# vressegu/sdeflow-light

Hardware: AMD Instinct MI355X
Metric: score-matching train steps/sec (+ reverse-SDE sample steps/sec) (higher is better)
Workload: dtype f32

## Files before the change

sdeflow_light_amd/csrc/attention_train_kernels.hip:

```cpp
#include "attention_common.h"

template <int CT, int QT, int KB, int NW = 4, bool MH = false>
__global__ void __launch_bounds__(64 * NW) k_attn_dual_fwd(const float* __restrict__ qkv, float* __restrict__ att,
                                                        float* __restrict__ lse, float* __restrict__ rbar, int T, int nqb,
                                                        int64_t Bp, float scale, int nh) {
  constexpr int C = 16 * CT, KP = C + 4, KT = KB / 16, NT = 64 * NW;
  constexpr int NV = (KB * C / 4) / NT;
  static_assert(NV >= 1 && (KB * C / 4) % NT == 0, "key block does not divide over the workgroup's threads");
  extern __shared__ __attribute__((aligned(16))) float atd_lds[];
  float* Ks = atd_lds;
  float* Kd = Ks + KB * KP;
  float* Vs = Kd + KB * KP;
  float* Vd = Vs + KB * KP;
  const int tid = threadIdx.x, w = tid >> 6, lane = tid & 63, il = lane & 15, q = lane >> 4;
  const int64_t NP = MH ? Bp * nh : Bp;
  int pr, qb;
  {
    const int full = (int)(NP / 8) * 8 * nqb, b = blockIdx.x;
    if (b < full) { const int loc = b >> 3; pr = (loc / nqb) * 8 + (b & 7); qb = loc % nqb; }
    else { const int r = b - full; pr = (int)(NP / 8) * 8 + r / nqb; qb = r % nqb; }
  }
  const AttnHead H = attn_head<MH, C>(pr, nh);
  const int LD = H.LD, LA = H.LA, smp = H.smp;
  const float* bp = qkv + (size_t)smp * T * LD + H.qcol;
  const float* bt = bp + (size_t)Bp * T * LD;
  const int q0 = (qb * NW + w) * 16 * QT;

  f32x4 qf[QT][CT], qd[QT][CT], o[QT][CT], od[QT][CT];
  float m[QT], l[QT], rr[QT];
#pragma unroll
  for (int qt = 0; qt < QT; ++qt) {
#pragma unroll
    for (int g = 0; g < CT; ++g) {
      const size_t off = (size_t)(q0 + 16 * qt + il) * LD + 16 * g + 4 * q;
      qf[qt][g] = *reinterpret_cast<const f32x4*>(bp + off);
      qd[qt][g] = *reinterpret_cast<const f32x4*>(bt + off);
      o[qt][g] = f32x4{0, 0, 0, 0};
      od[qt][g] = f32x4{0, 0, 0, 0};
    }
    m[qt] = -INFINITY; l[qt] = 0.f; rr[qt] = 0.f;
  }

  f32x4 pk[NV], pkd[NV], pv[NV], pvd[NV];
  auto gload = [&](int kb) __attribute__((always_inline)) {
#pragma unroll
    for (int i = 0; i < NV; ++i) {
      const int idx = tid + NT * i, key = idx / (C / 4), c4 = idx - key * (C / 4);
      const size_t off = (size_t)(kb * KB + key) * LD + 4 * c4;
      pk[i] = *reinterpret_cast<const f32x4*>(bp + off + C);
      pv[i] = *reinterpret_cast<const f32x4*>(bp + off + 2 * C);
      pkd[i] = *reinterpret_cast<const f32x4*>(bt + off + C);
      pvd[i] = *reinterpret_cast<const f32x4*>(bt + off + 2 * C);
    }
  };
  gload(0);
  const int nkb = T / KB;
  for (int kb = 0; kb < nkb; ++kb) {
    __syncthreads();
#pragma unroll
    for (int i = 0; i < NV; ++i) {
      const int idx = tid + NT * i, key = idx / (C / 4), c4 = idx - key * (C / 4);
      *reinterpret_cast<f32x4*>(Ks + key * KP + 4 * c4) = pk[i];
      *reinterpret_cast<f32x4*>(Kd + key * KP + 4 * c4) = pkd[i];
      *reinterpret_cast<f32x4*>(Vs + key * KP + 4 * c4) = pv[i];
      *reinterpret_cast<f32x4*>(Vd + key * KP + 4 * c4) = pvd[i];
    }
    __syncthreads();
    if (kb + 1 < nkb) gload(kb + 1);

    f32x4 s[QT][KT], sd[QT][KT];
#pragma unroll
    for (int kt = 0; kt < KT; ++kt) {
#pragma unroll
      for (int qt = 0; qt < QT; ++qt) { s[qt][kt] = f32x4{0, 0, 0, 0}; sd[qt][kt] = f32x4{0, 0, 0, 0}; }
#pragma unroll
      for (int g = 0; g < CT; ++g) {
        const f32x4 a = *reinterpret_cast<const f32x4*>(Ks + (16 * kt + il) * KP + 16 * g + 4 * q);
        const f32x4 ad = *reinterpret_cast<const f32x4*>(Kd + (16 * kt + il) * KP + 16 * g + 4 * q);
#pragma unroll
        for (int r = 0; r < 4; ++r)
#pragma unroll
          for (int qt = 0; qt < QT; ++qt) {
            s[qt][kt] = mfma16(a[r], qf[qt][g][r], s[qt][kt]);
            sd[qt][kt] = mfma16(a[r], qd[qt][g][r], sd[qt][kt]);
            sd[qt][kt] = mfma16(ad[r], qf[qt][g][r], sd[qt][kt]);
          }
      }
    }
#pragma unroll
    for (int qt = 0; qt < QT; ++qt) {
      float mb = -INFINITY;
#pragma unroll
      for (int kt = 0; kt < KT; ++kt)
#pragma unroll
        for (int r = 0; r < 4; ++r) { s[qt][kt][r] *= scale; mb = fmaxf(mb, s[qt][kt][r]); }
      mb = fmaxf(mb, __shfl_xor(mb, 16, 64));
      mb = fmaxf(mb, __shfl_xor(mb, 32, 64));
      const float mn = fmaxf(m[qt], mb);
      const float alpha = expf(m[qt] - mn);
      m[qt] = mn;
      float ls = 0.f, lr = 0.f;
#pragma unroll
      for (int kt = 0; kt < KT; ++kt)
#pragma unroll
        for (int r = 0; r < 4; ++r) {
          const float p = expf(s[qt][kt][r] - mn);
          const float wv = p * (sd[qt][kt][r] * scale);
          s[qt][kt][r] = p; sd[qt][kt][r] = wv;
          ls += p; lr += wv;
        }
      l[qt] = l[qt] * alpha + ls;
      rr[qt] = rr[qt] * alpha + lr;
#pragma unroll
      for (int ct = 0; ct < CT; ++ct) { o[qt][ct] *= alpha; od[qt][ct] *= alpha; }
    }
#pragma unroll
    for (int kt = 0; kt < KT; ++kt)
#pragma unroll
      for (int ct = 0; ct < CT; ++ct) {
        float a[4], ad[4];
#pragma unroll
        for (int r = 0; r < 4; ++r) {
          a[r] = Vs[(16 * kt + 4 * q + r) * KP + 16 * ct + il];
          ad[r] = Vd[(16 * kt + 4 * q + r) * KP + 16 * ct + il];
        }
#pragma unroll
        for (int r = 0; r < 4; ++r)
#pragma unroll
          for (int qt = 0; qt < QT; ++qt) {
            o[qt][ct] = mfma16(a[r], s[qt][kt][r], o[qt][ct]);
            od[qt][ct] = mfma16(a[r], sd[qt][kt][r], od[qt][ct]);
            od[qt][ct] = mfma16(ad[r], s[qt][kt][r], od[qt][ct]);
          }
      }
  }
#pragma unroll
  for (int qt = 0; qt < QT; ++qt) {
    float lt = l[qt], rt = rr[qt];
    lt += __shfl_xor(lt, 16, 64); lt += __shfl_xor(lt, 32, 64);
    rt += __shfl_xor(rt, 16, 64); rt += __shfl_xor(rt, 32, 64);
    const float inv = 1.0f / lt, rb = rt * inv;
    const size_t row = (size_t)smp * T + q0 + 16 * qt + il;
    float* orow = att + row * LA + H.acol;
    float* drow = att + ((size_t)Bp * T + row) * LA + H.acol;
#pragma unroll
    for (int ct = 0; ct < CT; ++ct) {
      const f32x4 ov = o[qt][ct] * inv;
      *reinterpret_cast<f32x4*>(orow + 16 * ct + 4 * q) = ov;
      *reinterpret_cast<f32x4*>(drow + 16 * ct + 4 * q) = od[qt][ct] * inv - ov * rb;
    }
    if (q == 0) {
      const size_t sr = (size_t)pr * T + q0 + 16 * qt + il;
      lse[sr] = m[qt] + logf(lt); rbar[sr] = rb;
    }
  }
}

template <bool MH = false>
__global__ void __launch_bounds__(256) k_attn_dual_delta(const float* __restrict__ att, const float* __restrict__ datt,
                                                          const float* __restrict__ rbar, float* __restrict__ cc,
                                                          float* __restrict__ de, int64_t rows, int C, int T, int nh) {
  const int64_t row = (int64_t)blockIdx.x * 16 + (threadIdx.x >> 4);
  const int sl = threadIdx.x & 15;
  float c = 0.f, d = 0.f;
  if (row < rows) {
    const size_t off = MH ? attn_mh_row(row / T, row % T, T, C, nh) : (size_t)row * C;
    const float* o = att + off;
    const float* g = datt + off;
    const float* od = att + (size_t)rows * C + off;
    const float* gd = datt + (size_t)rows * C + off;
    for (int c4 = sl; c4 < C / 4; c4 += 16) {
      const f32x4 ov = *reinterpret_cast<const f32x4*>(o + 4 * c4), gv = *reinterpret_cast<const f32x4*>(g + 4 * c4);
      const f32x4 odv = *reinterpret_cast<const f32x4*>(od + 4 * c4), gdv = *reinterpret_cast<const f32x4*>(gd + 4 * c4);
#pragma unroll
      for (int r = 0; r < 4; ++r) { c += gdv[r] * ov[r]; d += gv[r] * ov[r] + gdv[r] * odv[r]; }
    }
  }
#pragma unroll
  for (int s = 8; s > 0; s >>= 1) { c += __shfl_xor(c, s, 16); d += __shfl_xor(d, s, 16); }
  if (row < rows && sl == 0) { cc[row] = c; de[row] = d - rbar[row] * c; }
}

template <int CT, int KG, bool ACC = false, bool MH = false>
__global__ void __launch_bounds__(128 * KG) k_attn_dual_bwd(const float* __restrict__ qkv, const float* __restrict__ datt,
                                                        const float* __restrict__ stats ,
                                                        const float* __restrict__ ccde ,
                                                        float* __restrict__ dqkv, float* __restrict__ slab, int T, int nkg,
                                                        int kseq, int ks, int64_t Bp, float scale, int nh) {
  constexpr int C = 16 * CT, KP = C + 4, KB = 16 * KG, DP = KB + 4, QB = 32, NT = 128 * KG;
  constexpr int NK = (KB * C / 4 + NT - 1) / NT;
  constexpr bool KFULL = (KB * C / 4) % NT == 0;
  constexpr int NQ = (QB * C / 4 + NT - 1) / NT;
  constexpr bool QFULL = (QB * C / 4) % NT == 0;
  static_assert(NK >= 1 && NQ >= 1 && (KFULL || NK == 1) && (QFULL || NQ == 1), "tiles do not divide over the workgroup");
  const int64_t NP = MH ? Bp * nh : Bp;
  extern __shared__ __attribute__((aligned(16))) float atb_lds[];
  float* Ks = atb_lds;
  float* Kd = Ks + KB * KP;
  float* Vs = Kd + KB * KP;
  float* Vd = Vs + KB * KP;
  float* Qs = Vd + KB * KP;
  float* Qd = Qs + QB * KP;
  float* Gs = Qd + QB * KP;
  float* Gd = Gs + QB * KP;
  float* St = Gd + QB * KP;
  float* dS0 = St + 4 * QB;
  const int tid = threadIdx.x, w = tid >> 6, lane = tid & 63, il = lane & 15, q = lane >> 4;
  const int qs = w & 1, kg = w >> 1;
  int pr, kgi;
  {
    const int full = (int)(NP / 8) * 8 * nkg, b = blockIdx.x;
    if (b < full) { const int loc = b >> 3; pr = (loc / nkg) * 8 + (b & 7); kgi = loc % nkg; }
    else { const int r = b - full; pr = (int)(NP / 8) * 8 + r / nkg; kgi = r % nkg; }
  }
  const AttnHead H = attn_head<MH, C>(pr, nh);
  const int LD = H.LD, LA = H.LA, smp = H.smp;
  const int kb = kgi * kseq + ks;
  const size_t half_qkv = (size_t)Bp * T * LD, half_att = (size_t)Bp * T * LA;
  const float* bp = qkv + (size_t)smp * T * LD + H.qcol;
  const float* gp = datt + (size_t)smp * T * LA + H.acol;
  const size_t srow0 = (size_t)pr * T;

#pragma unroll
  for (int i = 0; i < NK; ++i) {
    const int idx = tid + NT * i, key = idx / (C / 4), c4 = idx - key * (C / 4);
    if (!KFULL && idx >= KB * C / 4) break;
    const size_t off = (size_t)(kb * KB + key) * LD + 4 * c4;
    *reinterpret_cast<f32x4*>(Ks + key * KP + 4 * c4) = *reinterpret_cast<const f32x4*>(bp + off + C);
    *reinterpret_cast<f32x4*>(Vs + key * KP + 4 * c4) = *reinterpret_cast<const f32x4*>(bp + off + 2 * C);
    *reinterpret_cast<f32x4*>(Kd + key * KP + 4 * c4) = *reinterpret_cast<const f32x4*>(bp + half_qkv + off + C);
    *reinterpret_cast<f32x4*>(Vd + key * KP + 4 * c4) = *reinterpret_cast<const f32x4*>(bp + half_qkv + off + 2 * C);
  }

  f32x4 dk[CT], dkd[CT], dv[CT], dvd[CT];
#pragma unroll
  for (int ct = 0; ct < CT; ++ct) dk[ct] = dkd[ct] = dv[ct] = dvd[ct] = f32x4{0, 0, 0, 0};

  f32x4 pq[NQ], pqd[NQ], pg[NQ], pgd[NQ];
  float pst = 0.f;
  auto gload = [&](int qb) __attribute__((always_inline)) {
#pragma unroll
    for (int i = 0; i < NQ; ++i) {
      const int idx = tid + NT * i, qr = idx / (C / 4), c4 = idx - qr * (C / 4);
      if (!QFULL && idx >= QB * C / 4) break;
      const size_t row = (size_t)(qb * QB + qr);
      pq[i] = *reinterpret_cast<const f32x4*>(bp + row * LD + 4 * c4);
      pqd[i] = *reinterpret_cast<const f32x4*>(bp + half_qkv + row * LD + 4 * c4);
      pg[i] = *reinterpret_cast<const f32x4*>(gp + row * LA + 4 * c4);
      pgd[i] = *reinterpret_cast<const f32x4*>(gp + half_att + row * LA + 4 * c4);
    }
    if (tid < 4 * QB) {
      const int which = tid >> 5, qr = tid & 31;
      const size_t o = (size_t)(which & 1) * (size_t)NP * T + srow0 + (size_t)qb * QB + qr;
      pst = which < 2 ? stats[o] : ccde[o];
    }
  };
  gload(0);
  const int nqb = T / QB;
  for (int qb = 0; qb < nqb; ++qb) {
    float* dS = dS0 + (qb & 1) * (2 * QB * DP);
    float* dSd = dS + QB * DP;
#pragma unroll
    for (int i = 0; i < NQ; ++i) {
      const int idx = tid + NT * i, qr = idx / (C / 4), c4 = idx - qr * (C / 4);
      if (!QFULL && idx >= QB * C / 4) break;
      *reinterpret_cast<f32x4*>(Qs + qr * KP + 4 * c4) = pq[i];
      *reinterpret_cast<f32x4*>(Qd + qr * KP + 4 * c4) = pqd[i];
      *reinterpret_cast<f32x4*>(Gs + qr * KP + 4 * c4) = pg[i];
      *reinterpret_cast<f32x4*>(Gd + qr * KP + 4 * c4) = pgd[i];
    }
    if (tid < 4 * QB) St[tid] = pst;
    __syncthreads();
    if (qb + 1 < nqb) gload(qb + 1);

    f32x4 s = {0, 0, 0, 0}, sd = {0, 0, 0, 0}, pb = {0, 0, 0, 0}, dd = {0, 0, 0, 0};
#pragma unroll
    for (int g = 0; g < CT; ++g) {
      const int ao = (16 * qs + il) * KP + 16 * g + 4 * q, bo = (16 * kg + il) * KP + 16 * g + 4 * q;
      const f32x4 aQ = *reinterpret_cast<const f32x4*>(Qs + ao), aQd = *reinterpret_cast<const f32x4*>(Qd + ao);
      const f32x4 aG = *reinterpret_cast<const f32x4*>(Gs + ao), aGd = *reinterpret_cast<const f32x4*>(Gd + ao);
      const f32x4 bK = *reinterpret_cast<const f32x4*>(Ks + bo), bKd = *reinterpret_cast<const f32x4*>(Kd + bo);
      const f32x4 bV = *reinterpret_cast<const f32x4*>(Vs + bo), bVd = *reinterpret_cast<const f32x4*>(Vd + bo);
#pragma unroll
      for (int r = 0; r < 4; ++r) {
        s = mfma16(aQ[r], bK[r], s);
        sd = mfma16(aQd[r], bK[r], sd);
        pb = mfma16(aG[r], bV[r], pb);
        dd = mfma16(aGd[r], bV[r], dd);
        sd = mfma16(aQ[r], bKd[r], sd);
        pb = mfma16(aGd[r], bVd[r], pb);
      }
      __builtin_amdgcn_sched_barrier(0);
    }
    const f32x4 L4 = *reinterpret_cast<const f32x4*>(St + 16 * qs + 4 * q);
    const f32x4 R4 = *reinterpret_cast<const f32x4*>(St + QB + 16 * qs + 4 * q);
    const f32x4 C4 = *reinterpret_cast<const f32x4*>(St + 2 * QB + 16 * qs + 4 * q);
    const f32x4 D4 = *reinterpret_cast<const f32x4*>(St + 3 * QB + 16 * qs + 4 * q);
    f32x4 p, pd, ds, dsd;
#pragma unroll
    for (int r = 0; r < 4; ++r) {
      const float sv = s[r] * scale, sdv = sd[r] * scale;
      const float pv = expf(sv - L4[r]), e = sdv - R4[r];
      p[r] = pv;
      pd[r] = pv * e;
      dsd[r] = pv * (dd[r] - C4[r]);
      ds[r] = pv * (pb[r] + dd[r] * e - C4[r] * sdv - D4[r]);
      dS[(16 * qs + 4 * q + r) * DP + 16 * kg + il] = ds[r];
      dSd[(16 * qs + 4 * q + r) * DP + 16 * kg + il] = dsd[r];
    }
#pragma unroll
    for (int ct = 0; ct < CT; ++ct) {
      float aG[4], aGd[4], aQ[4], aQd[4];
#pragma unroll
      for (int r = 0; r < 4; ++r) {
        const int o = (16 * qs + 4 * q + r) * KP + 16 * ct + il;
        aG[r] = Gs[o]; aGd[r] = Gd[o]; aQ[r] = Qs[o]; aQd[r] = Qd[o];
      }
#pragma unroll
      for (int r = 0; r < 4; ++r) {
        dv[ct] = mfma16(aG[r], p[r], dv[ct]);
        dvd[ct] = mfma16(aGd[r], p[r], dvd[ct]);
        dk[ct] = mfma16(aQ[r], ds[r], dk[ct]);
        dkd[ct] = mfma16(aQ[r], dsd[r], dkd[ct]);
        dv[ct] = mfma16(aGd[r], pd[r], dv[ct]);
        dk[ct] = mfma16(aQd[r], dsd[r], dk[ct]);
      }
      __builtin_amdgcn_sched_barrier(0);
    }
    __syncthreads();
#pragma unroll
    for (int ct = kg; ct < CT; ct += KG) {
      const size_t row = (size_t)qb * QB + 16 * qs + il;
      float* sp = slab + (((size_t)pr * nkg + kgi) * T + row) * C + 16 * ct + 4 * q;
      float* sdp = slab + (((size_t)(NP + pr) * nkg + kgi) * T + row) * C + 16 * ct + 4 * q;
      f32x4 dq = {0, 0, 0, 0}, dqd = {0, 0, 0, 0}, pdq = {0, 0, 0, 0}, pdqd = {0, 0, 0, 0};
      if (ACC) {
        pdq = *reinterpret_cast<const f32x4*>(sp);
        pdqd = *reinterpret_cast<const f32x4*>(sdp);
      }
#pragma unroll
      for (int kt = 0; kt < KG; ++kt) {
        const f32x4 b1 = *reinterpret_cast<const f32x4*>(dS + (16 * qs + il) * DP + 16 * kt + 4 * q);
        const f32x4 b2 = *reinterpret_cast<const f32x4*>(dSd + (16 * qs + il) * DP + 16 * kt + 4 * q);
        float a1[4], a2[4];
#pragma unroll
        for (int r = 0; r < 4; ++r) {
          a1[r] = Ks[(16 * kt + 4 * q + r) * KP + 16 * ct + il];
          a2[r] = Kd[(16 * kt + 4 * q + r) * KP + 16 * ct + il];
        }
#pragma unroll
        for (int r = 0; r < 4; ++r) {
          dq = mfma16(a1[r], b1[r], dq);
          dqd = mfma16(a1[r], b2[r], dqd);
          dq = mfma16(a2[r], b2[r], dq);
        }
      }
      if (ACC) { dq += pdq; dqd += pdqd; }
      *reinterpret_cast<f32x4*>(sp) = dq;
      *reinterpret_cast<f32x4*>(sdp) = dqd;
    }
  }
  __syncthreads();
  float* scratch = atb_lds;
  if (qs == 1) {
#pragma unroll
    for (int ct = 0; ct < CT; ++ct) {
      f32x4* base = reinterpret_cast<f32x4*>(scratch) + ((size_t)kg * 4 * CT + 4 * ct) * 64 + lane;
      base[0] = dk[ct]; base[64] = dkd[ct]; base[128] = dv[ct]; base[192] = dvd[ct];
    }
  }
  __syncthreads();
  if (qs == 0) {
    const size_t row = (size_t)smp * T + kb * KB + 16 * kg + il;
    float* kp_ = dqkv + row * LD + H.qcol;
    float* kt_ = dqkv + half_qkv + row * LD + H.qcol;
#pragma unroll
    for (int ct = 0; ct < CT; ++ct) {
      const f32x4* base = reinterpret_cast<const f32x4*>(scratch) + ((size_t)kg * 4 * CT + 4 * ct) * 64 + lane;
      *reinterpret_cast<f32x4*>(kp_ + C + 16 * ct + 4 * q) = (dk[ct] + base[0]) * scale;
      *reinterpret_cast<f32x4*>(kt_ + C + 16 * ct + 4 * q) = (dkd[ct] + base[64]) * scale;
      *reinterpret_cast<f32x4*>(kp_ + 2 * C + 16 * ct + 4 * q) = dv[ct] + base[128];
      *reinterpret_cast<f32x4*>(kt_ + 2 * C + 16 * ct + 4 * q) = dvd[ct] + base[192];
    }
  }
}

template <bool MH = false>
__global__ void __launch_bounds__(256) k_attn_dq_reduce(const float* __restrict__ slab, float* __restrict__ dqkv, int64_t N,
                                                         int T, int C, int nkb, float scale, int nh) {
  const int64_t total = N * T * (C / 4);
  for (int64_t i = (int64_t)blockIdx.x * 256 + threadIdx.x; i < total; i += (int64_t)gridDim.x * 256) {
    const int c4 = (int)(i % (C / 4));
    const int64_t row = i / (C / 4);
    const int64_t n = row / T, qr = row - n * T;
    const float* p = slab + ((size_t)n * nkb * T + qr) * C + 4 * c4;
    f32x4 acc = *reinterpret_cast<const f32x4*>(p);
    for (int kb = 1; kb < nkb; ++kb) acc += *reinterpret_cast<const f32x4*>(p + (size_t)kb * T * C);
    *reinterpret_cast<f32x4*>(dqkv + (MH ? attn_mh_row(n, qr, T, 3 * C, nh) : (size_t)row * 3 * C) + 4 * c4) = acc * scale;
  }
}

template <int CT, int QT, int KB, int NW, bool MH = false>
static int launch_fwd(const float* qkv, float* att, float* stats, int64_t Bp, int T, float scale, hipStream_t st, int nh = 1) {
  constexpr int C = 16 * CT;
  constexpr size_t lds = (size_t)4 * KB * (C + 4) * sizeof(float);
  static const int once = attn_allow_lds(&k_attn_dual_fwd<CT, QT, KB, NW, MH>, lds); (void)once;
  const int nqb = T / (16 * NW * QT);
  const int64_t NP = Bp * nh;
  hipLaunchKernelGGL((k_attn_dual_fwd<CT, QT, KB, NW, MH>), dim3((unsigned)(NP * nqb)), dim3(64 * NW), lds, st, qkv, att, stats,
                     stats + NP * T, T, nqb, Bp, scale, nh);
  return msgm_check_launch();
}

static inline int attn_bwd_keys(int C) { return C == 128 ? 32 : 64; }

template <int CT, int KG, bool MH = false>
static int launch_bwd(const float* qkv, const float* att, const float* datt, const float* stats, float* dqkv, int64_t Bp, int T,
                      float scale, float* ws, hipStream_t st, int nh = 1) {
  constexpr int C = 16 * CT, KP = C + 4, KB = 16 * KG;
  constexpr size_t lds_main = ((size_t)4 * KB * KP + 4 * 32 * KP + 4 * 32 + 4 * 32 * (KB + 4)) * sizeof(float);
  constexpr size_t lds_epi = (size_t)KG * 4 * CT * 64 * 4 * sizeof(float);
  constexpr size_t lds = lds_main > lds_epi ? lds_main : lds_epi;
  static_assert(lds <= 160 * 1024, "backward tiles exceed the CU's LDS");
  static const int once = attn_allow_lds(&k_attn_dual_bwd<CT, KG, false, MH>, lds) | attn_allow_lds(&k_attn_dual_bwd<CT, KG, true, MH>, lds);
  (void)once;
  const int64_t NP = Bp * nh;
  const int64_t rows = NP * T;
  const int nkb = T / KB;
  int kseq = 1;
  for (int k = 2; k > 1; k >>= 1)
    if (nkb % k == 0 && NP * (int64_t)(nkb / k) >= 1024) { kseq = k; break; }
  const int nkg = nkb / kseq;
  float* cc = ws;
  float* de = ws + rows;
  float* slab = ws + 2 * rows;
  hipLaunchKernelGGL(k_attn_dual_delta<MH>, dim3((unsigned)((rows + 15) / 16)), dim3(256), 0, st, att, datt, stats + rows, cc, de,
                     rows, C, T, nh);
  hipLaunchKernelGGL((k_attn_dual_bwd<CT, KG, false, MH>), dim3((unsigned)(NP * nkg)), dim3(128 * KG), lds, st, qkv, datt, stats, cc, dqkv,
                     slab, T, nkg, kseq, 0, Bp, scale, nh);
  for (int ks = 1; ks < kseq; ++ks)
    hipLaunchKernelGGL((k_attn_dual_bwd<CT, KG, true, MH>), dim3((unsigned)(NP * nkg)), dim3(128 * KG), lds, st, qkv, datt, stats, cc,
                       dqkv, slab, T, nkg, kseq, ks, Bp, scale, nh);
  const int64_t work = 2 * NP * T * (C / 4);
  hipLaunchKernelGGL(k_attn_dq_reduce<MH>, dim3((unsigned)grid_for(work, 256, 16384)), dim3(256), 0, st, slab, dqkv, 2 * NP, T, C,
                     nkg, scale, nh);
  return msgm_check_launch();
}

static bool attn_dual_ok(int32_t T, int32_t heads, int32_t D, bool mh) {
  if (heads < 1 || heads > 64) return false;
  if (D == 128) return T >= 32 && T % 32 == 0;
  return ((mh && D == 16) || D == 32 || D == 64) && T >= 64 && T % 64 == 0;
}

static size_t attn_dual_ws(int64_t Bp, int32_t T, int32_t heads, int32_t D, bool mh) {
  if (!attn_dual_ok(T, heads, D, mh) || Bp <= 0) return 0;
  const size_t np = (size_t)Bp * heads;
  return ((size_t)2 * np * T + (size_t)2 * np * (T / attn_bwd_keys(D)) * T * D) * sizeof(float);
}

template <bool MH>
static int attn_dual_fwd_go(const float* qkv, float* att, float* stats, int64_t Bp, int T, int D, int nh, float scale, hipStream_t st) {
  if (D == 128) {
    if (T % 64 == 0 && Bp * nh * (int64_t)(T / 64) >= 512) return launch_fwd<8, 1, 16, 4, MH>(qkv, att, stats, Bp, T, scale, st, nh);
    return launch_fwd<8, 1, 16, 2, MH>(qkv, att, stats, Bp, T, scale, st, nh);
  }
  if (D == 64) return launch_fwd<4, 1, 32, 4, MH>(qkv, att, stats, Bp, T, scale, st, nh);
  if (D == 32) return launch_fwd<2, 1, 64, 4, MH>(qkv, att, stats, Bp, T, scale, st, nh);
  if constexpr (MH) return launch_fwd<1, 1, 64, 4, MH>(qkv, att, stats, Bp, T, scale, st, nh);
  return MSGM_E_UNSUPPORTED;
}

template <bool MH>
static int attn_dual_bwd_go(const float* qkv, const float* att, const float* datt, const float* stats, float* dqkv, int64_t Bp, int T,
                            int D, int nh, float scale, float* ws, hipStream_t st) {
  if (D == 128) return launch_bwd<8, 2, MH>(qkv, att, datt, stats, dqkv, Bp, T, scale, ws, st, nh);
  if (D == 64) return launch_bwd<4, 4, MH>(qkv, att, datt, stats, dqkv, Bp, T, scale, ws, st, nh);
  if (D == 32) return launch_bwd<2, 4, MH>(qkv, att, datt, stats, dqkv, Bp, T, scale, ws, st, nh);
  if constexpr (MH) return launch_bwd<1, 4, MH>(qkv, att, datt, stats, dqkv, Bp, T, scale, ws, st, nh);
  return MSGM_E_UNSUPPORTED;
}

static int attn_dual_forward(const float* qkv, float* att, float* stats, int64_t Bp, int32_t T, int32_t heads, int32_t D, bool mh,
                             float scale, msgm_stream_t stream) {
  if (!qkv || !att || !stats || Bp <= 0 || T <= 0 || heads <= 0 || D <= 0) return MSGM_E_BADARG;
  if (!attn_dual_ok(T, heads, D, mh) || Bp * heads * (int64_t)(T / 32) > 0x7fffffffLL) return MSGM_E_UNSUPPORTED;
  if (!mh || (heads == 1 && attn_dual_ok(T, 1, D, false))) return attn_dual_fwd_go<false>(qkv, att, stats, Bp, T, D, 1, scale, S(stream));
  return attn_dual_fwd_go<true>(qkv, att, stats, Bp, T, D, heads, scale, S(stream));
}

static int attn_dual_backward(const float* qkv, const float* att, const float* datt, const float* stats, float* dqkv, int64_t Bp,
                              int32_t T, int32_t heads, int32_t D, bool mh, float scale, void* workspace, size_t workspace_bytes,
                              msgm_stream_t stream) {
  if (!qkv || !att || !datt || !stats || !dqkv || !workspace || Bp <= 0 || T <= 0 || heads <= 0 || D <= 0) return MSGM_E_BADARG;
  if (!attn_dual_ok(T, heads, D, mh) || Bp * heads * (int64_t)(T / 32) > 0x7fffffffLL) return MSGM_E_UNSUPPORTED;
  if (workspace_bytes < attn_dual_ws(Bp, T, heads, D, mh)) return MSGM_E_WORKSPACE;
  float* ws = static_cast<float*>(workspace);
  if (!mh || (heads == 1 && attn_dual_ok(T, 1, D, false))) return attn_dual_bwd_go<false>(qkv, att, datt, stats, dqkv, Bp, T, D, 1, scale, ws, S(stream));
  return attn_dual_bwd_go<true>(qkv, att, datt, stats, dqkv, Bp, T, D, heads, scale, ws, S(stream));
}

extern "C" {

int msgm_attention_dual_supported(int32_t T, int32_t C) { return attn_dual_ok(T, 1, C, false); }
int msgm_attention_dual_mh_supported(int32_t T, int32_t heads, int32_t D) { return attn_dual_ok(T, heads, D, true); }

size_t msgm_attention_dual_workspace(int64_t Bp, int32_t T, int32_t C) { return attn_dual_ws(Bp, T, 1, C, false); }
size_t msgm_attention_dual_mh_workspace(int64_t Bp, int32_t T, int32_t heads, int32_t D) { return attn_dual_ws(Bp, T, heads, D, true); }

int msgm_attention_dual_forward(const float* qkv, float* att, float* stats, int64_t Bp, int32_t T, int32_t C, float scale,
                                msgm_stream_t stream) {
  return attn_dual_forward(qkv, att, stats, Bp, T, 1, C, false, scale, stream);
}

int msgm_attention_dual_mh_forward(const float* qkv, float* att, float* stats, int64_t Bp, int32_t T, int32_t heads, int32_t D,
                                   float scale, msgm_stream_t stream) {
  return attn_dual_forward(qkv, att, stats, Bp, T, heads, D, true, scale, stream);
}

int msgm_attention_dual_backward(const float* qkv, const float* att, const float* datt, const float* stats, float* dqkv,
                                 int64_t Bp, int32_t T, int32_t C, float scale, void* workspace, size_t workspace_bytes,
                                 msgm_stream_t stream) {
  return attn_dual_backward(qkv, att, datt, stats, dqkv, Bp, T, 1, C, false, scale, workspace, workspace_bytes, stream);
}

int msgm_attention_dual_mh_backward(const float* qkv, const float* att, const float* datt, const float* stats, float* dqkv,
                                    int64_t Bp, int32_t T, int32_t heads, int32_t D, float scale, void* workspace,
                                    size_t workspace_bytes, msgm_stream_t stream) {
  return attn_dual_backward(qkv, att, datt, stats, dqkv, Bp, T, heads, D, true, scale, workspace, workspace_bytes, stream);
}

}
```

Measured before the change: 10.40.

## Software-pipeline LDS fragment reads and cache K columns in registers in dual attention backward

When CT equals KG, the dual attention backward kernel double-buffers its LDS fragment loads. The next channel group's Q/G/K/V row fragments and column fragments are read into registers while the current group's MFMAs run, with sched barriers to enforce the order. The K and Kd column fragments used for dQ are hoisted out of the query-block loop and kept in registers, and the dS tiles are preloaded before the dQ MFMAs. This targets LDS latency stalls between MFMA chains, at the cost of more VGPRs and possible lower occupancy.

```diff
diff --git a/sdeflow_light_amd/csrc/attention_train_kernels.hip b/sdeflow_light_amd/csrc/attention_train_kernels.hip
--- a/sdeflow_light_amd/csrc/attention_train_kernels.hip
+++ b/sdeflow_light_amd/csrc/attention_train_kernels.hip
@@ -179,6 +179,20 @@
 #pragma unroll
   for (int s = 8; s > 0; s >>= 1) { c += __shfl_xor(c, s, 16); d += __shfl_xor(d, s, 16); }
   if (row < rows && sl == 0) { cc[row] = c; de[row] = d - rbar[row] * c; }
+}
+
+
+template <int STRIDE>
+__device__ __forceinline__ void attn_rd_rows(const float* lds, int off, f32x4* f) {
+#pragma unroll
+  for (int m = 0; m < 4; ++m) f[m] = *reinterpret_cast<const f32x4*>(lds + off + m * STRIDE);
+}
+template <int STRIDE, int KP>
+__device__ __forceinline__ void attn_rd_cols(const float* lds, int off, float (*f)[4]) {
+#pragma unroll
+  for (int r = 0; r < 4; ++r)
+#pragma unroll
+    for (int m = 0; m < 4; ++m) f[m][r] = lds[off + m * STRIDE + r * KP];
 }
 
 template <int CT, int KG, bool ACC = false, bool MH = false>
@@ -236,6 +250,28 @@
 #pragma unroll
   for (int ct = 0; ct < CT; ++ct) dk[ct] = dkd[ct] = dv[ct] = dvd[ct] = f32x4{0, 0, 0, 0};
 
+  constexpr bool PF = CT == KG;
+  int fa = 0, fb = 0, fc = 0;
+  if constexpr (PF) {
+    int fa4 = KB * KP + (16 * qs + il) * (KP / 4) + q;
+    int fb4 = (16 * kg + il) * (KP / 4) + q;
+    fc = 4 * KB * KP + (16 * qs + 4 * q) * KP + il;
+    asm volatile("" : "+v"(fa4), "+v"(fb4), "+v"(fc));
+    fa = 4 * fa4;
+    fb = 4 * fb4;
+  }
+  float k1[PF ? KG : 1][4], k2[PF ? KG : 1][4];
+  if constexpr (PF) {
+    __syncthreads();
+#pragma unroll
+    for (int kt = 0; kt < KG; ++kt)
+#pragma unroll
+      for (int r = 0; r < 4; ++r) {
+        k1[kt][r] = Ks[(16 * kt + 4 * q + r) * KP + 16 * kg + il];
+        k2[kt][r] = Kd[(16 * kt + 4 * q + r) * KP + 16 * kg + il];
+      }
+  }
+
   f32x4 pq[NQ], pqd[NQ], pg[NQ], pgd[NQ];
   float pst = 0.f;
   auto gload = [&](int qb) __attribute__((always_inline)) {
@@ -270,17 +306,27 @@
       *reinterpret_cast<f32x4*>(Gd + qr * KP + 4 * c4) = pgd[i];
     }
     if (tid < 4 * QB) St[tid] = pst;
+    f32x4 A[PF ? 2 : 1][4], B[PF ? 2 : 1][4];
+    float cf[PF ? 2 : 1][4][4];
+    if constexpr (PF) attn_rd_rows<KB * KP>(atb_lds, fb, B[0]);
     __syncthreads();
+    if constexpr (PF) attn_rd_rows<QB * KP>(atb_lds, fa, A[0]);
     if (qb + 1 < nqb) gload(qb + 1);
 
     f32x4 s = {0, 0, 0, 0}, sd = {0, 0, 0, 0}, pb = {0, 0, 0, 0}, dd = {0, 0, 0, 0};
 #pragma unroll
     for (int g = 0; g < CT; ++g) {
+      const int c = PF ? g & 1 : 0;
+      if constexpr (PF) {
+        if (g + 1 < CT) { attn_rd_rows<QB * KP>(atb_lds + 16 * (g + 1), fa, A[c ^ 1]); attn_rd_rows<KB * KP>(atb_lds + 16 * (g + 1), fb, B[c ^ 1]); }
+        else attn_rd_cols<QB * KP, KP>(atb_lds, fc, cf[0]);
+        __builtin_amdgcn_sched_barrier(0);
+      }
       const int ao = (16 * qs + il) * KP + 16 * g + 4 * q, bo = (16 * kg + il) * KP + 16 * g + 4 * q;
-      const f32x4 aQ = *reinterpret_cast<const f32x4*>(Qs + ao), aQd = *reinterpret_cast<const f32x4*>(Qd + ao);
-      const f32x4 aG = *reinterpret_cast<const f32x4*>(Gs + ao), aGd = *reinterpret_cast<const f32x4*>(Gd + ao);
-      const f32x4 bK = *reinterpret_cast<const f32x4*>(Ks + bo), bKd = *reinterpret_cast<const f32x4*>(Kd + bo);
-      const f32x4 bV = *reinterpret_cast<const f32x4*>(Vs + bo), bVd = *reinterpret_cast<const f32x4*>(Vd + bo);
+      const f32x4 aQ = PF ? A[c][0] : *reinterpret_cast<const f32x4*>(Qs + ao), aQd = PF ? A[c][1] : *reinterpret_cast<const f32x4*>(Qd + ao);
+      const f32x4 aG = PF ? A[c][2] : *reinterpret_cast<const f32x4*>(Gs + ao), aGd = PF ? A[c][3] : *reinterpret_cast<const f32x4*>(Gd + ao);
+      const f32x4 bK = PF ? B[c][0] : *reinterpret_cast<const f32x4*>(Ks + bo), bKd = PF ? B[c][1] : *reinterpret_cast<const f32x4*>(Kd + bo);
+      const f32x4 bV = PF ? B[c][2] : *reinterpret_cast<const f32x4*>(Vs + bo), bVd = PF ? B[c][3] : *reinterpret_cast<const f32x4*>(Vd + bo);
 #pragma unroll
       for (int r = 0; r < 4; ++r) {
         s = mfma16(aQ[r], bK[r], s);
@@ -310,11 +356,17 @@
     }
 #pragma unroll
     for (int ct = 0; ct < CT; ++ct) {
+      const int c = PF ? ct & 1 : 0;
+      if constexpr (PF) {
+        if (ct + 1 < CT) attn_rd_cols<QB * KP, KP>(atb_lds + 16 * (ct + 1), fc, cf[c ^ 1]);
+        __builtin_amdgcn_sched_barrier(0);
+      }
       float aG[4], aGd[4], aQ[4], aQd[4];
 #pragma unroll
       for (int r = 0; r < 4; ++r) {
         const int o = (16 * qs + 4 * q + r) * KP + 16 * ct + il;
-        aG[r] = Gs[o]; aGd[r] = Gd[o]; aQ[r] = Qs[o]; aQd[r] = Qd[o];
+        aG[r] = PF ? cf[c][2][r] : Gs[o]; aGd[r] = PF ? cf[c][3][r] : Gd[o];
+        aQ[r] = PF ? cf[c][0][r] : Qs[o]; aQd[r] = PF ? cf[c][1][r] : Qd[o];
       }
 #pragma unroll
       for (int r = 0; r < 4; ++r) {
@@ -338,15 +390,24 @@
         pdq = *reinterpret_cast<const f32x4*>(sp);
         pdqd = *reinterpret_cast<const f32x4*>(sdp);
       }
+      f32x4 t1[PF ? KG : 1], t2[PF ? KG : 1];
+      if constexpr (PF) {
+#pragma unroll
+        for (int kt = 0; kt < KG; ++kt) {
+          t1[kt] = *reinterpret_cast<const f32x4*>(dS + (16 * qs + il) * DP + 16 * kt + 4 * q);
+          t2[kt] = *reinterpret_cast<const f32x4*>(dSd + (16 * qs + il) * DP + 16 * kt + 4 * q);
+        }
+        __builtin_amdgcn_sched_barrier(0);
+      }
 #pragma unroll
       for (int kt = 0; kt < KG; ++kt) {
-        const f32x4 b1 = *reinterpret_cast<const f32x4*>(dS + (16 * qs + il) * DP + 16 * kt + 4 * q);
-        const f32x4 b2 = *reinterpret_cast<const f32x4*>(dSd + (16 * qs + il) * DP + 16 * kt + 4 * q);
+        const f32x4 b1 = PF ? t1[PF ? kt : 0] : *reinterpret_cast<const f32x4*>(dS + (16 * qs + il) * DP + 16 * kt + 4 * q);
+        const f32x4 b2 = PF ? t2[PF ? kt : 0] : *reinterpret_cast<const f32x4*>(dSd + (16 * qs + il) * DP + 16 * kt + 4 * q);
         float a1[4], a2[4];
 #pragma unroll
         for (int r = 0; r < 4; ++r) {
-          a1[r] = Ks[(16 * kt + 4 * q + r) * KP + 16 * ct + il];
-          a2[r] = Kd[(16 * kt + 4 * q + r) * KP + 16 * ct + il];
+          a1[r] = PF ? k1[PF ? kt : 0][r] : Ks[(16 * kt + 4 * q + r) * KP + 16 * ct + il];
+          a2[r] = PF ? k2[PF ? kt : 0][r] : Kd[(16 * kt + 4 * q + r) * KP + 16 * ct + il];
         }
 #pragma unroll
         for (int r = 0; r < 4; ++r) {
```

New measurement: 10.51 (median of 6 runs). +1.1%, better.
